# yellofi/SelectiveNet_for_semantic_segmentation_binary

Hardware: AMD Instinct MI355X
Metric: train images/sec, SelectiveUNet_B 256x256 bs=128 (global), selective_loss s_lamb=2 (higher is better)
Workload: dtype f32; 1 GPU; SelectiveUNet_B train step, global bs=128, 256x256, Adam lr=1e-3, s_lamb=2; model=SelectiveUNet_B, global_batch=128, per_gpu_batch=128, image=256, parallelism=dp1

## Files before the change

### selectivenet_for_semantic_segmentation_binary_amd/csrc/conv3x3.hip

```cpp
#include <cstdlib>

#include "gemm_common.h"

namespace selunet {

constexpr int TH = 16, TW = 16;
constexpr int HHT = TH + 2, HWT = TW + 2;
constexpr int HPIX = HHT * HWT;
constexpr int HTHREADS = 512;
constexpr int A_ROUNDS = (HPIX * 8 + HTHREADS - 1) / HTHREADS;
constexpr int AROWB = 160;
__device__ __forceinline__ int halo_off(int hp, int cc) { return hp * AROWB + ((cc ^ ((hp / HWT) & 1)) << 4); }

template <typename T, int BN, bool ONE_CHUNK>
__global__ void __launch_bounds__(HTHREADS, ONE_CHUNK ? 2 : 1)
conv3x3_halo_kernel(GatherArg g, const T* __restrict__ B, int N, int k_pad, EpiArg ep, int n_tiles, int tiles_x,
                    int tiles_y) {
  constexpr int E = 16 / sizeof(T);
  constexpr int CK = 128 / sizeof(T);
  constexpr int WAVES_N = BN / 64;
  constexpr int WAVES_M = 8 / WAVES_N;
  constexpr int WPIX = (TH * TW) / WAVES_M;
  constexpr int MT = WPIX / 32;
  constexpr int NT = 2;
// ... 290 lines not shown
        h[e] = a;
        l[e] = b;
      }
      const int par = (hp / HWT) & 1;
      *reinterpret_cast<f16x4*>(base + (((cc >> 1) ^ par) << 4) + (cc & 1) * 8) = h;
      *reinterpret_cast<f16x4*>(base + (((4 + (cc >> 1)) ^ par) << 4) + (cc & 1) * 8) = l;
    } else {
      *reinterpret_cast<uint4*>(base + (((cc ^ ((hp / HWT) & 1))) << 4)) = v;
    }
  };

  auto halo_store_prepped = [&](int hb, int hp, int cc, uint4 v) __attribute__((always_inline)) {
    unsigned char* base = As + hb * HPIX * AROWB + hp * AROWB;
    if constexpr (X2) {
      const int par = (hp / HWT) & 1;
      *reinterpret_cast<uint2*>(base + (((cc >> 1) ^ par) << 4) + (cc & 1) * 8) = make_uint2(v.x, v.y);
      *reinterpret_cast<uint2*>(base + (((4 + (cc >> 1)) ^ par) << 4) + (cc & 1) * 8) = make_uint2(v.z, v.w);
    } else {
      *reinterpret_cast<uint4*>(base + (((cc ^ ((hp / HWT) & 1))) << 4)) = v;
    }
  };
  auto tile_xy = [&](int pt_i, int& img, int& y0, int& x0) __attribute__((always_inline)) {
    const unsigned pt = (unsigned)pt_i;
    const unsigned r = pt / (unsigned)tiles_x;
    x0 = (int)(pt - r * (unsigned)tiles_x) * TW;
    const unsigned r2 = r / (unsigned)tiles_y;
    y0 = (int)(r - r2 * (unsigned)tiles_y) * TH;
    img = (int)r2;
  };
  auto a_slot = [&](int round, int& hp, int& cc) -> bool {
    const int hidx = round * HTHREADS + tid;
    hp = min(hidx >> 3, HPIX - 1);
    cc = hidx & 7;
    return hidx < HPIX * 8;
  };
  auto a_inside = [&](int y0, int x0, int hp) -> bool {
    const int hy = hp / HWT, hx = hp - (hp / HWT) * HWT;
    return (unsigned)(y0 - 1 + hy) < (unsigned)g.h && (unsigned)(x0 - 1 + hx) < (unsigned)g.w;
  };
  auto chunk_src = [&](int chunk, int& c) -> SrcArg {
    c = chunk * CK;
    const bool s1 = g.nsrc > 1 && c >= g.src[0].C;
    if (s1) c -= g.src[0].C;
    return pick_src(g, s1 ? 1 : 0);
  };
  auto a_ptr = [&](const SrcArg& sa, int c, int img, int y0, int x0, int hp, int cc) -> const uint4* {
    const int hy = hp / HWT, hx = hp - (hp / HWT) * HWT;
    const int ys = min(max(y0 - 1 + hy, 0), g.h - 1), xs = min(max(x0 - 1 + hx, 0), g.w - 1);
    return reinterpret_cast<const uint4*>(reinterpret_cast<const T*>(sa.data) +
                                          (((int64_t)img * g.h + ys) * g.w + xs) * sa.C + c + cc * E);
  };
  constexpr int XRPIX = 3 * HWT;
  static_assert(!X2 || (A_ROUNDS * 3 == HHT && XRPIX * 8 <= HTHREADS), "three halo rows per round");
  const int xq = tid >> 3, xcc = tid & 7;
  const int xhp = xq < XRPIX ? xq : xq - XRPIX;
  const int xry = (xhp >= HWT) + (xhp >= 2 * HWT), xhx = xhp - xry * HWT;
  const unsigned xpix = (unsigned)(xry * g.w + xhx);
  const unsigned xb_off = (unsigned)(xq * k_pad * 4 + xcc * 16);
  const unsigned xb_rstride = (unsigned)(64 * k_pad * 4);
  auto x_lds = [](int t) __attribute__((always_inline)) {
    const int q = t >> 3, cc = t & 7, hp = q < XRPIX ? q : q - XRPIX;
    const int ry = (hp >= HWT) + (hp >= 2 * HWT);
    return (unsigned)(hp * AROWB + (((cc >> 1) ^ (ry & 1)) << 4) + (cc & 1) * 8);
  };
  const unsigned xlds = x_lds(tid);
  unsigned xtb = 0;
  if constexpr (X2) {
    const int hrem = g.h - (tiles_y - 1) * TH, wrem = g.w - (tiles_x - 1) * TW;
#pragma unroll
    for (int r = 0; r < A_ROUNDS; ++r) {
      const int hy = 3 * r + xry;
      xtb |= (unsigned)((hy == 0) | (hy > hrem) << 6 | (xhx == 0) << 12 | (xhx > wrem) << 18) << r;
    }
  }
  struct Geo {
    int img, y0, x0;
    int64_t pix;
    unsigned em;
  };
  auto tile_geo = [&](int pt_) __attribute__((always_inline)) {
    const unsigned pt = (unsigned)__builtin_amdgcn_readfirstlane(pt_);
    const unsigned r = pt / (unsigned)tiles_x, tx = pt - r * (unsigned)tiles_x;
    const unsigned r2 = r / (unsigned)tiles_y, ty = r - r2 * (unsigned)tiles_y;
    Geo q;
    q.img = (int)r2;
    q.y0 = (int)ty * TH;
    q.x0 = (int)tx * TW;
    q.pix = ((int64_t)r2 * g.h + ty * TH) * g.w + tx * TW;
    q.em = (ty == 0 ? 0x3fu : 0u) | (ty == (unsigned)tiles_y - 1u ? 0x3fu << 6 : 0u) |
           (tx == 0 ? 0x3fu << 12 : 0u) | (tx == (unsigned)tiles_x - 1u ? 0x3fu << 18 : 0u);
    return q;
  };
  struct XStage {
    int64_t e0;
    unsigned off, rstride, safe, out;
  };
  auto x_stage = [&](const Geo& q, const SrcArg& sa, int c) __attribute__((always_inline)) {
    XStage s;
    s.e0 = (q.pix - g.w - 1) * sa.C + c;
    s.off = __umul24(xpix, (unsigned)sa.C * 4u) + (unsigned)xcc * 16u;
    s.rstride = (unsigned)(3 * g.w * sa.C) * 4u;
    s.safe = (unsigned)((g.w + 1) * sa.C) * 4u;
    s.out = xtb & q.em;
    return s;
  };
  auto x_out = [](const XStage& s, int r) __attribute__((always_inline)) { return (s.out & (0x41041u << r)) != 0; };
  auto at = [](const void* base, int64_t elems, unsigned off) __attribute__((always_inline)) {
    return reinterpret_cast<const uint4*>(
        reinterpret_cast<const char*>(reinterpret_cast<const float*>(base) + elems) + (size_t)off);
  };
  auto x_load = [&](const XStage& s, const SrcArg& sa, int r) __attribute__((always_inline)) {
    unsigned rs = (unsigned)r * s.rstride;
    asm volatile("" : "+s"(rs));
    return *at(sa.data, s.e0, x_out(s, r) ? s.safe : s.off + rs);
  };
  auto x_split4 = [&](uint4 v) __attribute__((always_inline)) {
#ifdef SELUNET_ABL_RAW_HALO
    return v;
#else
    float f[4];
    __builtin_memcpy(f, &v, 16);
    f16x4 h, l;
#pragma unroll
    for (int e = 0; e < 4; ++e) {
      _Float16 a, b;
      x2_split(f[e] * xs, a, b);
      h[e] = a;
      l[e] = b;
    }
    uint4 o;
    __builtin_memcpy(&o.x, &h, 8);
    __builtin_memcpy(&o.z, &l, 8);
    return o;
#endif
  };
  auto x_put = [&](int hb, int r, unsigned lds, uint4 o) __attribute__((always_inline)) {
    unsigned char* p = As + hb * HPIX * AROWB + r * (XRPIX * AROWB) + (lds ^ ((unsigned)(r & 1) << 4));
    *reinterpret_cast<uint2*>(p) = make_uint2(o.x, o.y);
    *reinterpret_cast<uint2*>(p + 64) = make_uint2(o.z, o.w);
  };
  struct BRegs {
    uint4 v[B_ROUNDS];
  };
  auto b_load = [&](int st) __attribute__((always_inline)) {
    const int chunk = st / 9, tap = st - chunk * 9;
    const int k0 = tap * g.Ctot + chunk * CK;
    BRegs rb;
    if constexpr (X2) {
      const int64_t e0 = (int64_t)n0 * k_pad + k0;
      unsigned o = xb_off;
      asm volatile("" : "+v"(o));
#pragma unroll
      for (int r = 0; r < B_ROUNDS; ++r) rb.v[r] = *at(B, e0, o + (unsigned)r * xb_rstride);
      return rb;
    }
#pragma unroll
    for (int r = 0; r < B_ROUNDS; ++r) {
      const int idx = r * HTHREADS + tid;
      const int row = idx >> 3, cc = idx & 7;
      rb.v[r] = *reinterpret_cast<const uint4*>(B + (int64_t)(n0 + row) * k_pad + k0 + cc * E);
    }
    return rb;
  };
  auto b_store = [&](const BRegs& rb, int buf) __attribute__((always_inline)) {
#pragma unroll
    for (int r = 0; r < B_ROUNDS; ++r) {
      const int idx = r * HTHREADS + tid;
      const int row = idx >> 3, cc = idx & 7;
      *reinterpret_cast<uint4*>(Bs + (buf * BN + row) * WROWB + cc * 16) = rb.v[r];
    }
  };

  AccT acc[AM][AN];
#pragma unroll
  for (int a = 0; a < AM; ++a)
#pragma unroll
    for (int b = 0; b < AN; ++b) acc[a][b] = AccT{};
  int hrow0[MT], hsw0[MT];
#pragma unroll
  for (int a = 0; a < MT; ++a) {
    const int pix = wm * WPIX + a * 32 + l32;
    hrow0[a] = (pix / TW) * HWT + (pix % TW);
    hsw0[a] = half ^ ((pix / TW) & 1);
  }
  auto mma_step = [&](int hbuf, int bbuf, int t) __attribute__((always_inline)) {
    const unsigned char* a_src = As + hbuf * HPIX * AROWB;
    const unsigned char* b_src = Bs + bbuf * BN * WROWB;
    const int dy = t / 3, dx = t - (t / 3) * 3;
    const int tap_off = dy * HWT + dx;
    if constexpr (M16) {
      f16x8 bh[4], bl[4];
#pragma unroll
      for (int b = 0; b < 4; ++b) {
        const unsigned char* p = b_src + (wn * 64 + b * 16 + l16) * WROWB + kg * 16;
        bh[b] = *reinterpret_cast<const f16x8*>(p);
        bl[b] = *reinterpret_cast<const f16x8*>(p + 64);
      }
#pragma unroll
      for (int a = 0; a < RT; ++a) {
        const int py = wm * RT + a;
        const unsigned char* p =
            a_src + ((py + dy) * HWT + l16 + dx) * AROWB + ((kg ^ ((py + dy) & 1)) << 4);
        const f16x8 ah = *reinterpret_cast<const f16x8*>(p);
        const f16x8 al = *reinterpret_cast<const f16x8*>(p + 64);
#pragma unroll
        for (int b = 0; b < 4; ++b) {
          acc[a][b] = __builtin_amdgcn_mfma_f32_16x16x32_f16(ah, bl[b], acc[a][b], 0, 0, 0);
          acc[a][b] = __builtin_amdgcn_mfma_f32_16x16x32_f16(al, bh[b], acc[a][b], 0, 0, 0);
          acc[a][b] = __builtin_amdgcn_mfma_f32_16x16x32_f16(ah, bh[b], acc[a][b], 0, 0, 0);
        }
      }
    } else if constexpr (X2) {
#pragma unroll
      for (int ks = 0; ks < 2; ++ks) {
        f16x8 ah[MT], al[MT], bh[NT], bl[NT];
#pragma unroll
        for (int a = 0; a < MT; ++a) {
          const unsigned char* p = a_src + (hrow0[a] + tap_off) * AROWB + ((hsw0[a] ^ dy) & 1) * 16;
          ah[a] = *reinterpret_cast<const f16x8*>(p + ks * 32);
          al[a] = *reinterpret_cast<const f16x8*>(p + (2 + ks) * 32);
        }
#pragma unroll
        for (int b = 0; b < NT; ++b) {
          const unsigned char* p = b_src + (wn * 64 + b * 32 + l32) * ROWB + half * 16;
          bh[b] = *reinterpret_cast<const f16x8*>(p + ks * 32);
          bl[b] = *reinterpret_cast<const f16x8*>(p + (2 + ks) * 32);
        }
#pragma unroll
        for (int a = 0; a < MT; ++a)
#pragma unroll
          for (int b = 0; b < NT; ++b) {
            acc[a][b] = __builtin_amdgcn_mfma_f32_32x32x16_f16(ah[a], bl[b], acc[a][b], 0, 0, 0);
            acc[a][b] = __builtin_amdgcn_mfma_f32_32x32x16_f16(al[a], bh[b], acc[a][b], 0, 0, 0);
            acc[a][b] = __builtin_amdgcn_mfma_f32_32x32x16_f16(ah[a], bh[b], acc[a][b], 0, 0, 0);
          }
      }
    } else {
#pragma unroll
      for (int q = 0; q < 4; ++q) {
        const int boff = q * 32 + half * 16;
        uint4 af[MT], bfr[NT];
#pragma unroll
        for (int a = 0; a < MT; ++a)
          af[a] = *reinterpret_cast<const uint4*>(a_src + (hrow0[a] + tap_off) * AROWB + q * 32 + ((hsw0[a] ^ dy) & 1) * 16);
#pragma unroll
        for (int b = 0; b < NT; ++b)
          bfr[b] = *reinterpret_cast<const uint4*>(b_src + (wn * 64 + b * 32 + l32) * WROWB + boff);
#pragma unroll
        for (int a = 0; a < MT; ++a)
#pragma unroll
          for (int b = 0; b < NT; ++b) Mma<T>::run(acc[a][b], af[a], bfr[b]);
      }
    }
  };
  auto halo_put_global = [&](uint4 v, int r, const SrcArg& sa, int c, int y0, int x0, int hb)
      __attribute__((always_inline)) {
    int hp, cc;
    if (!a_slot(r, hp, cc)) return;
    uint4 o = make_uint4(0, 0, 0, 0);
    if (a_inside(y0, x0, hp)) o = sa.scale ? transform16<T>(v, sa.scale, sa.shift, c + cc * E, sa.relu) : v;
    halo_store(hb, hp, cc, o);
  };

  Geo gc{}, gn{};
  if constexpr (X2) gc = gn = tile_geo(TQ ? pt_cur : prow);
  if (!TQ || pt_cur < ptiles) {
    int c0;
    const SrcArg sa = chunk_src(0, c0);
    uint4 v0[A_ROUNDS];
    if constexpr (X2) {
      const XStage s0 = x_stage(gc, sa, c0);
#pragma unroll
      for (int r = 0; r < A_ROUNDS; ++r) v0[r] = x_load(s0, sa, r);
#pragma unroll
      for (int r = 0; r < A_ROUNDS; ++r) {
        uint4 o = make_uint4(0, 0, 0, 0);
        if (!x_out(s0, r)) o = sa.scale ? transform16<T>(v0[r], sa.scale, sa.shift, c0 + xcc * E, sa.relu) : v0[r];
        x_put(0, r, xlds, x_split4(o));
      }
    } else {
      int img, y0, x0;
      tile_xy(TQ ? pt_cur : prow, img, y0, x0);
#pragma unroll
      for (int r = 0; r < A_ROUNDS; ++r) {
        int hp, cc;
        a_slot(r, hp, cc);
        v0[r] = *a_ptr(sa, c0, img, y0, x0, hp, cc);
      }
#pragma unroll
      for (int r = 0; r < A_ROUNDS; ++r) halo_put_global(v0[r], r, sa, c0, y0, x0, 0);
    }
  }
  BRegs rb_next = b_load(0);
  b_store(rb_next, 0);
  rb_next = b_load(1 % csteps);
  __syncthreads();

  using Acc = std::conditional_t<X2 && BN == 128, float, typename StatAcc<T>::type>;
  static_assert(stats_flush_bytes<BN, HTHREADS, Acc>() <= (int)sizeof(smem), "statistics scratch exceeds LDS");
  Acc s1[8] = {0, 0, 0, 0, 0, 0, 0, 0}, s2[8] = {0, 0, 0, 0, 0, 0, 0, 0}, s3[8] = {0, 0, 0, 0, 0, 0, 0, 0};
  float amx = 0.0f;
  const TileStats ts = tile_stats(ep, TQ ? 0 : prow, n0, N);
  float* tile = reinterpret_cast<float*>(smem);
  uint4 ra[A_ROUNDS];
  int J = 0;
  int S = 0;
  unsigned claimed = 0;
  for (int i = 0; TQ ? pt_cur < ptiles : i < ntl; ++i) {
    int img, y0, x0;
    if constexpr (X2) {
      img = gc.img, y0 = gc.y0, x0 = gc.x0;
      if constexpr (!TQ) gn = i + 1 < ntl ? tile_geo(prow + (i + 1) * gp) : gc;
    } else {
      tile_xy(TQ ? pt_cur : prow + i * gp, img, y0, x0);
    }
    BRegs rb_hold;
    for (int c = 0; c < nchunks; ++c, ++J) {
      if constexpr (TQ) {
        if (c == 1) {
          pt_next = tq_slot;
          gn = pt_next < ptiles ? tile_geo(pt_next) : gc;
        }
      }
      const bool last_c = c + 1 == nchunks;
      const bool has_next = !last_c || (TQ ? pt_next < ptiles : i + 1 < ntl);
      const bool defer = last_c && has_next;
      int nimg = img, ny0 = y0, nx0 = x0;
      if constexpr (!X2) {
        if (defer) tile_xy(TQ ? pt_next : prow + (i + 1) * gp, nimg, ny0, nx0);
      }
      const int nc = !has_next ? c : (last_c ? 0 : c + 1);
      int cs;
      const SrcArg sn = chunk_src(nc, cs);
      XStage sx{};
      if constexpr (X2) sx = x_stage(defer ? gn : gc, sn, cs);
      float* ssc = Ss + ((J + 1) & 1) * CK;
      float* ssh = Ss + 2 * CK + ((J + 1) & 1) * CK;
      float coef = 0.0f;
#pragma unroll
      for (int t = 0; t < 9; ++t) {
        const int st2 = c * 9 + t + 2;
        const BRegs rb_far = b_load(st2 < csteps ? st2 : st2 - csteps);
        if (t == 0 && sn.scale && tid < 2 * CK) coef = tid < CK ? sn.scale[cs + tid] : sn.shift[cs + tid - CK];
#pragma unroll
        for (int r = 0; r < A_ROUNDS; ++r) {
          if (halo_load_tap(r) == t) {
            if constexpr (X2) {
              ra[r] = x_load(sx, sn, r);
            } else {
              int hp, cc;
              a_slot(r, hp, cc);
              ra[r] = *a_ptr(sn, cs, nimg, ny0, nx0, hp, cc);
            }
          }
        }
        if constexpr (TQ) {
          if (c == 0 && t == 0 && tid == 0) claimed = atomicAdd(tq + n_tile, 1u);
        }
        mma_step(J & 1, S & 1, t);
        if constexpr (TQ) {
          if (c == 0 && t == 8 && tid == 0) tq_slot = (int)min(claimed, (unsigned)ptiles);
        }
        if (defer && t == 8) rb_hold = rb_next;
        else b_store(rb_next, (S + 1) & 1);
        if (t == 1 && sn.scale && tid < 2 * CK) (tid < CK ? ssc[tid] : ssh[tid - CK]) = coef;
#pragma unroll
        for (int r = 0; r < A_ROUNDS; ++r) {
          if (halo_write_tap(r) != t) continue;
          if constexpr (X2) {
            uint4 v = ra[r];
#ifndef SELUNET_ABL_RAW_HALO
            if (sn.scale) {
              float e[4];
              __builtin_memcpy(e, &v, 16);
#pragma unroll
              for (int j = 0; j < 4; ++j) {
                float f = e[j] * ssc[xcc * 4 + j] + ssh[xcc * 4 + j];
                if (sn.relu) f = fmaxf(f, 0.0f);
                e[j] = f;
              }
              __builtin_memcpy(&v, e, 16);
            }
            if (x_out(sx, r)) v = make_uint4(0, 0, 0, 0);
#endif
            const uint4 o = x_split4(v);
            if (!defer) x_put((J + 1) & 1, r, xlds, o);
            else ra[r] = o;
            continue;
          }
          int hp, cc;
          if (a_slot(r, hp, cc)) {
            uint4 v = make_uint4(0, 0, 0, 0);
            if (a_inside(ny0, nx0, hp)) {
              v = ra[r];
              if (sn.scale) {
                T e[E];
                __builtin_memcpy(e, &v, 16);
#pragma unroll
                for (int j = 0; j < E; ++j) {
                  float f = to_f(e[j]) * ssc[cc * E + j] + ssh[cc * E + j];
                  if (sn.relu) f = fmaxf(f, 0.0f);
                  e[j] = from_f<T>(f);
                }
                __builtin_memcpy(&v, e, 16);
              }
            }
            if (!defer) {
              halo_store((J + 1) & 1, hp, cc, v);
            } else {
              if constexpr (X2) {
                float f[4];
                __builtin_memcpy(f, &v, 16);
                f16x4 h, l;
#pragma unroll
                for (int e = 0; e < 4; ++e) {
                  _Float16 a, b;
                  x2_split(f[e] * xs, a, b);
                  h[e] = a;
                  l[e] = b;
                }
                __builtin_memcpy(&v.x, &h, 8);
                __builtin_memcpy(&v.z, &l, 8);
              }
              ra[r] = v;
            }
          }
        }
        __syncthreads();
        rb_next = rb_far;
        ++S;
      }
      if (defer) {
      }
    }

    if constexpr (X2) {
#pragma unroll
      for (int a = 0; a < AM; ++a)
#pragma unroll
        for (int b = 0; b < AN; ++b) acc[a][b] *= cfac[b];
    }
    if constexpr (M16) {
#pragma unroll
      for (int a = 0; a < RT; ++a)
#pragma unroll
        for (int b = 0; b < 4; ++b)
#pragma unroll
          for (int i = 0; i < 4; ++i)
            tile[(wm * WPIX + a * 16 + 4 * kg + i) * (BN + 4) + wn * 64 + b * 16 + l16] = acc[a][b][i];
    } else {
      acc_to_lds<MT, NT, BN>(tile, acc, wm * WPIX, wn * 64, lane);
    }
#pragma unroll
    for (int a = 0; a < AM; ++a)
#pragma unroll
      for (int b = 0; b < AN; ++b) acc[a][b] = AccT{};
    __syncthreads();
    auto dst = [&](int pix, int cl) -> T* {
      const int y = y0 + pix / TW, x = x0 + pix % TW;
      if (y >= g.h || x >= g.w) return nullptr;
      const int64_t m = ((int64_t)img * g.h + y) * g.w + x;
      const int col = n0 + cl;
      if (ep.mode == SELUNET_EP_SPLIT)
        return col < ep.split ? reinterpret_cast<T*>(ep.out0) + m * ep.split + col
                              : reinterpret_cast<T*>(ep.out1) + m * (N - ep.split) + (col - ep.split);
      return reinterpret_cast<T*>(ep.out0) + m * N + col;
    };
    auto bias_col = [&](int cl) { return n0 + cl; };
    if constexpr (TQ) {
      TileStats tt = tile_stats(ep, pt_cur, n0, N);
      lds_tile_store_acc<T, TH * TW, BN, HTHREADS>(tile, tid, dst, ep.bias, bias_col, tt, s1, s2, s3, amx);
      tt.amax = nullptr;
      tile_stats_flush<BN, HTHREADS>(tile, tid, tt, s1, s2, s3, 0.0f);
#pragma unroll
      for (int e = 0; e < 8; ++e) s1[e] = s2[e] = s3[e] = 0;
    } else {
      lds_tile_store_acc<T, TH * TW, BN, HTHREADS>(tile, tid, dst, ep.bias, bias_col, ts, s1, s2, s3, amx);
    }
    if (TQ ? pt_next < ptiles : i + 1 < ntl) {
      __syncthreads();
      int tid2 = tid;
      asm volatile("" : "+v"(tid2));
#pragma unroll
      for (int r = 0; r < A_ROUNDS; ++r) {
        if constexpr (X2) {
          x_put(J & 1, r, x_lds(tid2), ra[r]);
        } else {
          const int hidx = r * HTHREADS + tid2;
          if (hidx < HPIX * 8) halo_store_prepped(J & 1, hidx >> 3, hidx & 7, ra[r]);
        }
      }
      b_store(rb_hold, S & 1);
      __syncthreads();
    }
    if constexpr (TQ) pt_cur = pt_next;
    gc = gn;
  }
  if constexpr (TQ) {
    if (ts.amax) block_amax(ts.amax, amx, tile);
    if (tid == 0 && atomicAdd(tq + n_tiles + n_tile, 1u) == (unsigned)gp - 1u) {
      atomicExch(tq + n_tile, 0u);
      atomicExch(tq + n_tiles + n_tile, 0u);
    }
  } else {
    tile_stats_flush<BN, HTHREADS>(tile, tid, ts, s1, s2, s3, amx);
  }
}

constexpr int WINO_STEPS = 12;
__device__ __forceinline__ int wino_row(int hp) {
  const int hy = hp / HWT, hx = hp - hy * HWT;
  return hy * HWT + (hx & 1) * (HWT / 2) + (hx >> 1);
}

template <int BN, int XS>
__global__ void __launch_bounds__(HTHREADS, 1)
conv3x3_wino_persist_kernel(GatherArg g, const float* __restrict__ B, int N, int k_pad, EpiArg ep, int n_tiles,
                            int tiles_x, int tiles_y, int ptiles, int gp) {
  using T = float;
  constexpr int E = 4;
  constexpr int CK = 32;
  constexpr int NT = BN / 64;
  constexpr int STEPS = WINO_STEPS / XS;
  constexpr int BROWS = XS * BN;
  constexpr int B_ROUNDS = BROWS * 8 / HTHREADS;
  static_assert(XS == 1 || XS == 2, "one or two planes per step");
  auto lt = [](int r) { return XS == 1 ? r : r >> 1; };
  static_assert(B_ROUNDS * HTHREADS == BROWS * 8, "weight tile rows must split evenly over the threads");
  static_assert(A_ROUNDS <= 6, "halo slice schedule covers six slices");

  constexpr int SMEM_MAIN = 2 * HPIX * AROWB + 2 * BROWS * ROWB + 2 * CK * 8;
  constexpr int SMEM_EPI = TH * TW * (BN + 4) * 4;
  __shared__ __attribute__((aligned(16))) unsigned char smem[SMEM_MAIN > SMEM_EPI ? SMEM_MAIN : SMEM_EPI];
  unsigned char* As = smem;
  unsigned char* Bs = smem + 2 * HPIX * AROWB;
  float* Ss = reinterpret_cast<float*>(Bs + 2 * BROWS * ROWB);

  const int tid = threadIdx.x;
  const int lane = tid & 63, wave = tid >> 6;
  const int wm = wave >> 1, wn = wave & 1;
  const int half = lane >> 5, l32 = lane & 31;
  const int pair = wm * 32 + l32, py = pair >> 3, px2 = pair & 7;

  const unsigned lb = xcd_remap(blockIdx.x, gridDim.x);
  const int n_tile = lb % n_tiles;
  const int prow = lb / n_tiles;
  const int n0 = n_tile * BN;
  const int ntl = prow < ptiles ? (ptiles - prow + gp - 1) / gp : 0;
  const int nchunks = g.Ctot / CK;
  const int csteps = nchunks * STEPS;

  auto tile_xy = [&](int i, int& img, int& y0, int& x0) __attribute__((always_inline)) {
    const unsigned pt = (unsigned)(prow + i * gp);
    const unsigned r = pt / (unsigned)tiles_x;
    x0 = (int)(pt - r * (unsigned)tiles_x) * TW;
    const unsigned r2 = r / (unsigned)tiles_y;
    y0 = (int)(r - r2 * (unsigned)tiles_y) * TH;
    img = (int)r2;
  };
  auto a_slot = [&](int round, int& hp, int& cc) -> bool {
    const int hidx = round * HTHREADS + tid;
    hp = min(hidx >> 3, HPIX - 1);
    cc = hidx & 7;
    return hidx < HPIX * 8;
  };
  auto a_inside = [&](int y0, int x0, int hp) -> bool {
    const int hy = hp / HWT, hx = hp - (hp / HWT) * HWT;
    return (unsigned)(y0 - 1 + hy) < (unsigned)g.h && (unsigned)(x0 - 1 + hx) < (unsigned)g.w;
  };
  auto chunk_src = [&](int chunk, int& c) -> SrcArg {
    c = chunk * CK;
    const bool s1 = g.nsrc > 1 && c >= g.src[0].C;
    if (s1) c -= g.src[0].C;
    return pick_src(g, s1 ? 1 : 0);
  };
  auto a_ptr = [&](const SrcArg& sa, int c, int img, int y0, int x0, int hp, int cc) -> const uint4* {
    const int hy = hp / HWT, hx = hp - (hp / HWT) * HWT;
    const int ys = min(max(y0 - 1 + hy, 0), g.h - 1), xs = min(max(x0 - 1 + hx, 0), g.w - 1);
    return reinterpret_cast<const uint4*>(reinterpret_cast<const T*>(sa.data) +
                                          (((int64_t)img * g.h + ys) * g.w + xs) * sa.C + c + cc * E);
  };
  struct BRegs {
    uint4 v[B_ROUNDS];
  };
  auto b_load = [&](int st) __attribute__((always_inline)) {
    const int chunk = st / STEPS, t = st - chunk * STEPS;
    BRegs rb;
#pragma unroll
    for (int r = 0; r < B_ROUNDS; ++r) {
      const int idx = r * HTHREADS + tid;
      const int row = idx >> 3, cc = idx & 7;
      const int pl = row / BN, co = row - pl * BN;
      const int k0 = (t * XS + pl) * g.Ctot + chunk * CK;
      rb.v[r] = *reinterpret_cast<const uint4*>(B + (int64_t)(n0 + co) * k_pad + k0 + cc * E);
    }
    return rb;
  };
  auto b_store = [&](const BRegs& rb, int buf) __attribute__((always_inline)) {
#pragma unroll
    for (int r = 0; r < B_ROUNDS; ++r) {
      const int idx = r * HTHREADS + tid;
      const int row = idx >> 3, cc = idx & 7;
      *reinterpret_cast<uint4*>(Bs + (buf * BROWS + row) * ROWB + cc * 16) = rb.v[r];
    }
  };

  f32x16 acc[4][NT];
#pragma unroll
  for (int x = 0; x < 4; ++x)
#pragma unroll
    for (int b = 0; b < NT; ++b) acc[x][b] = f32x16{};
  const int prow0 = py * HWT + px2;

  auto mma_step = [&](int hbuf, int bbuf, int t) __attribute__((always_inline)) {
    const unsigned char* a_src = As + hbuf * HPIX * AROWB;
    const unsigned char* b_src = Bs + bbuf * BROWS * ROWB;
    const int dy = (t * XS) >> 2, x0i = (t * XS) & 3;
    const int sw = ((half ^ (py + dy)) & 1) * 16;
    auto drow = [&](int j) { return a_src + (prow0 + dy * HWT + (j & 1) * (HWT / 2) + (j >> 1)) * AROWB + sw; };
#pragma unroll
    for (int q = 0; q < 4; ++q) {
      uint4 bfr[XS][NT];
#pragma unroll
      for (int p = 0; p < XS; ++p)
#pragma unroll
        for (int b = 0; b < NT; ++b)
          bfr[p][b] = *reinterpret_cast<const uint4*>(b_src + (p * BN + wn * (BN / 2) + b * 32 + l32) * ROWB + q * 32 +
                                                      half * 16);
      float4 v[XS];
      if (XS == 1) {
        const int xi = x0i;
        const int ja = xi == 0 ? 0 : (xi == 2 ? 2 : 1);
        const int jb = xi == 3 ? 3 : (xi == 2 ? 1 : 2);
        const float4 da = *reinterpret_cast<const float4*>(drow(ja) + q * 32);
        const float4 db = *reinterpret_cast<const float4*>(drow(jb) + q * 32);
        v[0] = xi == 1 ? make_float4(da.x + db.x, da.y + db.y, da.z + db.z, da.w + db.w)
                       : make_float4(da.x - db.x, da.y - db.y, da.z - db.z, da.w - db.w);
      } else {
        const int j0 = x0i == 0 ? 0 : 1;
        const float4 e0 = *reinterpret_cast<const float4*>(drow(j0) + q * 32);
        const float4 e1 = *reinterpret_cast<const float4*>(drow(j0 + 1) + q * 32);
        const float4 e2 = *reinterpret_cast<const float4*>(drow(j0 + 2) + q * 32);
        if (x0i == 0) {
          v[0] = make_float4(e0.x - e2.x, e0.y - e2.y, e0.z - e2.z, e0.w - e2.w);
          v[XS - 1] = make_float4(e1.x + e2.x, e1.y + e2.y, e1.z + e2.z, e1.w + e2.w);
        } else {
          v[0] = make_float4(e1.x - e0.x, e1.y - e0.y, e1.z - e0.z, e1.w - e0.w);
          v[XS - 1] = make_float4(e0.x - e2.x, e0.y - e2.y, e0.z - e2.z, e0.w - e2.w);
        }
      }
#pragma unroll
      for (int p = 0; p < XS; ++p) {
        const uint4 av = make_uint4(__float_as_uint(v[p].x), __float_as_uint(v[p].y), __float_as_uint(v[p].z),
                                    __float_as_uint(v[p].w));
#pragma unroll
        for (int b = 0; b < NT; ++b) Mma<float>::run(acc[x0i + p][b], av, bfr[p][b]);
      }
    }
  };
  auto halo_put_global = [&](uint4 v, int r, const SrcArg& sa, int c, int y0, int x0, int hb)
      __attribute__((always_inline)) {
    int hp, cc;
    if (!a_slot(r, hp, cc)) return;
    uint4 o = make_uint4(0, 0, 0, 0);
    if (a_inside(y0, x0, hp)) o = sa.scale ? transform16<T>(v, sa.scale, sa.shift, c + cc * E, sa.relu) : v;
    *reinterpret_cast<uint4*>(As + hb * HPIX * AROWB + halo_off(wino_row(hp), cc)) = o;
  };

  {
    int img, y0, x0;
    tile_xy(0, img, y0, x0);
    int c0;
    const SrcArg sa = chunk_src(0, c0);
    uint4 v0[A_ROUNDS];
#pragma unroll
    for (int r = 0; r < A_ROUNDS; ++r) {
      int hp, cc;
      a_slot(r, hp, cc);
      v0[r] = *a_ptr(sa, c0, img, y0, x0, hp, cc);
    }
#pragma unroll
    for (int r = 0; r < A_ROUNDS; ++r) halo_put_global(v0[r], r, sa, c0, y0, x0, 0);
  }
  BRegs rb_next = b_load(0);
  b_store(rb_next, 0);
  rb_next = b_load(1 % csteps);
  __syncthreads();

  using Acc = std::conditional_t<BN == 128, float, typename StatAcc<T>::type>;
  static_assert(stats_flush_bytes<BN, HTHREADS, Acc>() <= (int)sizeof(smem), "statistics scratch exceeds LDS");
  Acc s1[8] = {0, 0, 0, 0, 0, 0, 0, 0}, s2[8] = {0, 0, 0, 0, 0, 0, 0, 0}, s3[8] = {0, 0, 0, 0, 0, 0, 0, 0};
  float amx = 0.0f;
  const TileStats ts = tile_stats(ep, prow, n0, N);
  float* tile = reinterpret_cast<float*>(smem);
  uint4 ra[A_ROUNDS];
  int J = 0;
  int S = 0;
  for (int i = 0; i < ntl; ++i) {
    int img, y0, x0;
    tile_xy(i, img, y0, x0);
    BRegs rb_hold;
    for (int c = 0; c < nchunks; ++c, ++J) {
      const bool last_c = c + 1 == nchunks;
      const bool has_next = !last_c || i + 1 < ntl;
      const bool defer = last_c && has_next;
      int nimg = img, ny0 = y0, nx0 = x0;
      if (defer) tile_xy(i + 1, nimg, ny0, nx0);
      const int nc = !has_next ? c : (last_c ? 0 : c + 1);
      int cs;
      const SrcArg sn = chunk_src(nc, cs);
      float* ssc = Ss + ((J + 1) & 1) * CK;
      float* ssh = Ss + 2 * CK + ((J + 1) & 1) * CK;
      float coef = 0.0f;
#pragma unroll
      for (int t = 0; t < STEPS; ++t) {
        const int st2 = c * STEPS + t + 2;
        const BRegs rb_far = b_load(st2 < csteps ? st2 : st2 - csteps);
        if (t == 0 && !defer && sn.scale && tid < 2 * CK) coef = tid < CK ? sn.scale[cs + tid] : sn.shift[cs + tid - CK];
#pragma unroll
        for (int r = 0; r < A_ROUNDS; ++r) {
          if (lt(r) == t) {
            int hp, cc;
            a_slot(r, hp, cc);
            ra[r] = *a_ptr(sn, cs, nimg, ny0, nx0, hp, cc);
          }
        }
        mma_step(J & 1, S & 1, t);
        if (defer && t == STEPS - 1) rb_hold = rb_next;
        else b_store(rb_next, (S + 1) & 1);
        if (!defer) {
          if (t == 1 && sn.scale && tid < 2 * CK) (tid < CK ? ssc[tid] : ssh[tid - CK]) = coef;
#pragma unroll
          for (int r = 0; r < A_ROUNDS; ++r) {
            if (lt(r) + 3 != t) continue;
            int hp, cc;
            if (a_slot(r, hp, cc)) {
              uint4 v = make_uint4(0, 0, 0, 0);
              if (a_inside(ny0, nx0, hp)) {
                v = ra[r];
                if (sn.scale) {
                  float e[E];
                  __builtin_memcpy(e, &v, 16);
#pragma unroll
                  for (int j = 0; j < E; ++j) {
                    float f = e[j] * ssc[cc * E + j] + ssh[cc * E + j];
                    if (sn.relu) f = fmaxf(f, 0.0f);
                    e[j] = f;
                  }
                  __builtin_memcpy(&v, e, 16);
                }
              }
              *reinterpret_cast<uint4*>(As + ((J + 1) & 1) * HPIX * AROWB + halo_off(wino_row(hp), cc)) = v;
            }
          }
        }
        __syncthreads();
        rb_next = rb_far;
        ++S;
      }
    }

#pragma unroll
    for (int b = 0; b < NT; ++b) {
      const int col = wn * (BN / 2) + b * 32 + l32;
#pragma unroll
      for (int r = 0; r < 16; ++r) {
        const int pr = wm * 32 + (r & 3) + 8 * (r >> 2) + 4 * half;
        const int e = (pr >> 3) * TW + 2 * (pr & 7);
        const float m0 = acc[0][b][r], m1 = acc[1][b][r], m2 = acc[2][b][r], m3 = acc[3][b][r];
        tile[e * (BN + 4) + col] = (m0 + m1) + m2;
        tile[(e + 1) * (BN + 4) + col] = (m1 - m2) - m3;
      }
    }
#pragma unroll
    for (int x = 0; x < 4; ++x)
#pragma unroll
      for (int b = 0; b < NT; ++b) acc[x][b] = f32x16{};
    __syncthreads();
    auto dst = [&](int pix, int cl) -> T* {
      const int y = y0 + pix / TW, x = x0 + pix % TW;
// ... 1420 lines not shown
```

### selectivenet_for_semantic_segmentation_binary_amd/csrc/gemm_common.h

```cpp
#pragma once

#include <type_traits>

#include "common.h"

namespace selunet {

struct SrcArg {
  const void* data;
  const float* scale;
  const float* shift;
  int C;
  int relu;
  int layout;
  int pad;
};

struct GatherArg {
  int n, h, w;
  int taps;
  int nsrc;
  int Ctot;
  int hs, ws;
  int K;
  int small;
  int64_t M;
  SrcArg src[2];
};

__device__ __forceinline__ SrcArg pick_src(const GatherArg& g, int s) {
  SrcArg r;
  r.data = s ? g.src[1].data : g.src[0].data;
  r.scale = s ? g.src[1].scale : g.src[0].scale;
  r.shift = s ? g.src[1].shift : g.src[0].shift;
  r.C = s ? g.src[1].C : g.src[0].C;
  r.relu = s ? g.src[1].relu : g.src[0].relu;
  r.layout = s ? g.src[1].layout : g.src[0].layout;
  r.pad = 0;
  return r;
}

constexpr int BM = SELUNET_GEMM_BM;
constexpr int ROWB = 144;

__device__ __forceinline__ void tap_offset(int taps, int tap, int& dy, int& dx) {
  if (taps == 9) {
    dy = tap / 3 - 1;
    dx = tap - (tap / 3) * 3 - 1;
  } else if (taps == 4) {
    dy = tap >> 1;
    dx = tap & 1;
  } else {
    dy = 0;
    dx = 0;
  }
}

__device__ __forceinline__ bool src_pixel(const GatherArg& g, int tap, int y, int x, int& ys, int& xs) {
  int dy, dx;
  tap_offset(g.taps, tap, dy, dx);
  if (g.taps == 4) {
    ys = 2 * y + dy;
    xs = 2 * x + dx;
    return true;
  }
  ys = y + dy;
  xs = x + dx;
  return (unsigned)ys < (unsigned)g.hs && (unsigned)xs < (unsigned)g.ws;
}

__device__ __forceinline__ int64_t src_index(const GatherArg& g, int64_t m, int tap) {
  if (g.taps == 1) return m;
  const unsigned mu = (unsigned)m;
  const unsigned x = mu % (unsigned)g.w, t = mu / (unsigned)g.w;
  const unsigned y = t % (unsigned)g.h, img = t / (unsigned)g.h;
  int ys, xs;
  if (!src_pixel(g, tap, (int)y, (int)x, ys, xs)) return -1;
  return ((int64_t)img * g.hs + ys) * g.ws + xs;
}

template <typename T>
__device__ __forceinline__ float gather_scalar(const GatherArg& g, int64_t m, int k) {
  if (m >= g.M || k >= g.K) return 0.0f;
  const int tap = k / g.Ctot;
  int c = k - tap * g.Ctot;
  int s = 0;
  if (g.nsrc > 1 && c >= g.src[0].C) {
    c -= g.src[0].C;
    s = 1;
  }
  const int x = (int)(m % g.w);
  const int64_t t = m / g.w;
  const int y = (int)(t % g.h);
  const int img = (int)(t / g.h);
  int ys, xs;
  if (!src_pixel(g, tap, y, x, ys, xs)) return 0.0f;
  const SrcArg sa = pick_src(g, s);
  float v;
  if (sa.layout == 1) {
    v = reinterpret_cast<const float*>(sa.data)[(((int64_t)img * sa.C + c) * g.hs + ys) * g.ws + xs];
  } else {
    v = to_f(reinterpret_cast<const T*>(sa.data)[(((int64_t)img * g.hs + ys) * g.ws + xs) * sa.C + c]);
  }
  if (sa.scale) {
    v = v * sa.scale[c] + sa.shift[c];
    if (sa.relu) v = fmaxf(v, 0.0f);
  }
  return v;
}

template <typename T> struct Mma;
template <> struct Mma<float> {
  __device__ static inline void run(f32x16& acc, uint4 a, uint4 b) {
    acc = __builtin_amdgcn_mfma_f32_32x32x2f32(__uint_as_float(a.x), __uint_as_float(b.x), acc, 0, 0, 0);
    acc = __builtin_amdgcn_mfma_f32_32x32x2f32(__uint_as_float(a.y), __uint_as_float(b.y), acc, 0, 0, 0);
    acc = __builtin_amdgcn_mfma_f32_32x32x2f32(__uint_as_float(a.z), __uint_as_float(b.z), acc, 0, 0, 0);
    acc = __builtin_amdgcn_mfma_f32_32x32x2f32(__uint_as_float(a.w), __uint_as_float(b.w), acc, 0, 0, 0);
  }
};
template <> struct Mma<__bf16> {
  __device__ static inline void run(f32x16& acc, uint4 a, uint4 b) {
    bf16x8 av = __builtin_bit_cast(bf16x8, a);
    bf16x8 bv = __builtin_bit_cast(bf16x8, b);
    acc = __builtin_amdgcn_mfma_f32_32x32x16_bf16(av, bv, acc, 0, 0, 0);
  }
};

template <typename T>
__device__ __forceinline__ uint4 transform16(uint4 raw, const float* scale, const float* shift, int c, int relu) {
  constexpr int E = 16 / sizeof(T);
  T v[E];
  __builtin_memcpy(v, &raw, 16);
#pragma unroll
  for (int e = 0; e < E; ++e) {
    float f = to_f(v[e]) * scale[c + e] + shift[c + e];
    if (relu) f = fmaxf(f, 0.0f);
    v[e] = from_f<T>(f);
  }
  uint4 out;
  __builtin_memcpy(&out, v, 16);
  return out;
}

struct BnBwdArg {
  const void* y;
  const float* scale;
  const float* shift;
  const float* mean;
  const float* invstd;
  float* slab;
};

struct EpiArg {
  void* out0;
  void* out1;
  const float* bias;
  float* stats;
  int mode;
  int split;
  float* colsum;
  BnBwdArg bnb;
  float* amax;
  const float* stats_center;
};

typedef short s16x4 __attribute__((ext_vector_type(4)));

__device__ __forceinline__ unsigned xcd_remap(unsigned b, unsigned nb) {
  const unsigned xcd = b & 7u, q = nb >> 3, r = nb & 7u;
  const unsigned base = xcd < r ? xcd * (q + 1) : r * (q + 1) + (xcd - r) * q;
  return base + (b >> 3);
}

template <int MT, int NT, int TC>
__device__ __forceinline__ void acc_to_lds(float* tile, const f32x16 (&acc)[MT][NT], int wr0, int wc0, int lane) {
  const int half = lane >> 5, l32 = lane & 31;
#pragma unroll
  for (int a = 0; a < MT; ++a)
#pragma unroll
    for (int b = 0; b < NT; ++b)
#pragma unroll
      for (int r = 0; r < 16; ++r)
        tile[(wr0 + a * 32 + (r & 3) + 8 * (r >> 2) + 4 * half) * (TC + 4) + wc0 + b * 32 + l32] = acc[a][b][r];
}

struct TileStats {
  float* stats;
  int ld;
  float* colsum;
  int colsum_cols;
  int gcol0;
  BnBwdArg bnb;
  const void* out0;
  float* amax;
  const float* center;
};

__device__ __forceinline__ TileStats tile_stats(const EpiArg& ep, int64_t row, int n0, int N) {
  TileStats ts;
  ts.ld = N;
  ts.stats = ep.stats ? ep.stats + row * 2 * N + n0 : nullptr;
  ts.colsum = ep.colsum ? ep.colsum + row * ep.split + n0 : nullptr;
  ts.colsum_cols = ep.split;
  ts.gcol0 = n0;
  ts.bnb = ep.bnb;
  if (ep.bnb.slab) {
    ts.bnb.scale += n0;
    ts.bnb.shift += n0;
    ts.bnb.mean += n0;
    ts.bnb.invstd += n0;
    ts.bnb.slab += row * 3 * N + n0;
  }
  ts.out0 = ep.out0;
  ts.amax = ep.amax;
  ts.center = ep.stats_center ? ep.stats_center + n0 : nullptr;
  return ts;
}

template <typename T> struct StatAcc { using type = float; };
template <> struct StatAcc<float> { using type = double; };

template <typename T, int TR, int TC, int NTHREADS, typename Dst, typename BiasCol, typename Acc>
__device__ __forceinline__ void lds_tile_store_acc(float* tile, int tid, Dst&& dst, const float* bias,
                                                   BiasCol&& bias_col, const TileStats& ts, Acc (&s1)[8],
                                                   Acc (&s2)[8], Acc (&s3)[8], float& am) {
  constexpr int CC = TC / 8;
  constexpr int RS = NTHREADS / CC;
  asm volatile("" : "+v"(tid));
  const int cc = tid % CC, r0 = tid / CC;
  const int col = cc * 8;
  float bv[8], cen[8];
#pragma unroll
  for (int e = 0; e < 8; ++e) bv[e] = bias ? bias[bias_col(col + e)] : 0.0f;
  const bool do_st = ts.stats != nullptr;
#pragma unroll
  for (int e = 0; e < 8; ++e) cen[e] = do_st && ts.center ? ts.center[col + e] : 0.0f;
  const bool do_cs = ts.colsum != nullptr && ts.gcol0 + col < ts.colsum_cols;
  const bool do_bn = ts.bnb.slab != nullptr;
  float sc[8], sh[8], mu[8], is[8];
  if (do_bn) {
#pragma unroll
    for (int e = 0; e < 8; ++e) {
      sc[e] = ts.bnb.scale[col + e];
      sh[e] = ts.bnb.shift[col + e];
      mu[e] = ts.bnb.mean[col + e];
      is[e] = ts.bnb.invstd[col + e];
    }
  }
  __builtin_amdgcn_s_waitcnt(0x0F70);
  constexpr bool WIDE = !std::is_same<Acc, float>::value;
  float tw1[WIDE ? 8 : 1] = {}, tw2[WIDE ? 8 : 1] = {}, tw3[WIDE ? 8 : 1] = {};
  float* t1 = WIDE ? tw1 : reinterpret_cast<float*>(s1);
  float* t2 = WIDE ? tw2 : reinterpret_cast<float*>(s2);
  float* t3 = WIDE ? tw3 : reinterpret_cast<float*>(s3);
  constexpr int NR = TR / RS;
  constexpr int YB = NR < (TC >= 128 ? 4 : 2) ? NR : (TC >= 128 ? 4 : 2);
  static_assert(TR % RS == 0 && NR % YB == 0, "epilogue rows must split evenly over the threads");
#pragma unroll 1
  for (int rb = 0; rb < NR; rb += YB) {
  T yb[YB][8];
  if (do_bn) {
#pragma unroll
    for (int j = 0; j < YB; ++j) {
      const T* p = dst(r0 + (rb + j) * RS, col);
      if (p == nullptr) continue;
      const T* yp = reinterpret_cast<const T*>(ts.bnb.y) + (p - reinterpret_cast<const T*>(ts.out0));
      if constexpr (sizeof(T) == 2) {
        const uint4 u = *reinterpret_cast<const uint4*>(yp);
        __builtin_memcpy(yb[j], &u, 16);
      } else {
        const f32x4 a = *reinterpret_cast<const f32x4*>(yp), b = *reinterpret_cast<const f32x4*>(yp + 4);
        __builtin_memcpy(yb[j], &a, 16);
        __builtin_memcpy(yb[j] + 4, &b, 16);
      }
    }
  }
#pragma unroll
  for (int j = 0; j < YB; ++j) {
    const int row = r0 + (rb + j) * RS;
    T* p = dst(row, col);
    if (p == nullptr) continue;
    const f32x4 lo = *reinterpret_cast<const f32x4*>(tile + row * (TC + 4) + col);
    const f32x4 hi = *reinterpret_cast<const f32x4*>(tile + row * (TC + 4) + col + 4);
    float v[8] = {lo[0], lo[1], lo[2], lo[3], hi[0], hi[1], hi[2], hi[3]};
    if (do_st) {
#pragma unroll
      for (int e = 0; e < 8; ++e) {
        const float d = v[e] - cen[e];
        t1[e] += d;
        t2[e] += d * d;
      }
    }
#pragma unroll
    for (int e = 0; e < 8; ++e) v[e] += bv[e];
    T o[8];
#pragma unroll
    for (int e = 0; e < 8; ++e) o[e] = from_f<T>(v[e]);
    if (ts.amax) {
#pragma unroll
      for (int e = 0; e < 8; ++e) am = fmaxf(am, fabsf(to_f(o[e])));
    }
    if constexpr (sizeof(T) == 2) {
      uint4 u;
      __builtin_memcpy(&u, o, 16);
      *reinterpret_cast<uint4*>(p) = u;
    } else {
      *reinterpret_cast<f32x4*>(p) = f32x4{v[0], v[1], v[2], v[3]};
      *reinterpret_cast<f32x4*>(p + 4) = f32x4{v[4], v[5], v[6], v[7]};
    }
    if (do_cs) {
#pragma unroll
      for (int e = 0; e < 8; ++e) t1[e] += to_f(o[e]);
    }
    if (do_bn) {
#pragma unroll
      for (int e = 0; e < 8; ++e) {
        const float y = to_f(yb[j][e]);
        const float da = y * sc[e] + sh[e] > 0.0f ? to_f(o[e]) : 0.0f;
        const float xh = (y - mu[e]) * is[e];
        t1[e] += da;
        t2[e] += da * xh;
        t3[e] += xh;
      }
    }
  }
  }
  if constexpr (WIDE) {
#pragma unroll
    for (int e = 0; e < 8; ++e) {
      s1[e] += (Acc)t1[e];
      s2[e] += (Acc)t2[e];
      s3[e] += (Acc)t3[e];
    }
  }
}

template <int TC, int NTHREADS, typename Acc>
constexpr int stats_flush_bytes() { return (NTHREADS / (TC / 8)) * TC * 3 * (int)sizeof(Acc); }

template <int TC, int NTHREADS, typename Acc>
__device__ __forceinline__ void tile_stats_flush(float* red_f, int tid, const TileStats& ts, const Acc (&s1)[8],
                                                 const Acc (&s2)[8], const Acc (&s3)[8], float am) {
  constexpr int CC = TC / 8;
  constexpr int RS = NTHREADS / CC;
  Acc* red = reinterpret_cast<Acc*>(red_f);
  const int cc = tid % CC, r0 = tid / CC;
  const int col = cc * 8;
  const bool do_st = ts.stats != nullptr;
  const bool do_bn = ts.bnb.slab != nullptr;
  const int nst = do_bn ? 3 : (do_st ? 2 : 1);
  if (do_st || ts.colsum != nullptr || do_bn) {
    __syncthreads();
#pragma unroll
    for (int e = 0; e < 8; ++e) {
      red[(r0 * TC + col + e) * 3 + 0] = s1[e];
      red[(r0 * TC + col + e) * 3 + 1] = s2[e];
      red[(r0 * TC + col + e) * 3 + 2] = s3[e];
    }
    __syncthreads();
    for (int i = tid; i < TC * nst; i += NTHREADS) {
      const int c = i % TC, k = i / TC;
      Acc a = 0;
      for (int r = 0; r < RS; ++r) a += red[(r * TC + c) * 3 + k];
      if (do_bn) ts.bnb.slab[k * ts.ld + c] = a;
      else if (do_st) ts.stats[k * ts.ld + c] = a;
      else if (ts.gcol0 + c < ts.colsum_cols) ts.colsum[c] = a;
    }
  }
  if (ts.amax) block_amax(ts.amax, am, red_f);
}

template <typename T, int TR, int TC, int NTHREADS, typename Dst, typename BiasCol>
__device__ __forceinline__ void lds_tile_store(float* tile, int tid, Dst&& dst, const float* bias, BiasCol&& bias_col,
                                               const TileStats& ts) {
  float s1[8] = {0, 0, 0, 0, 0, 0, 0, 0}, s2[8] = {0, 0, 0, 0, 0, 0, 0, 0}, s3[8] = {0, 0, 0, 0, 0, 0, 0, 0};
  float am = 0.0f;
  lds_tile_store_acc<T, TR, TC, NTHREADS>(tile, tid, dst, bias, bias_col, ts, s1, s2, s3, am);
  tile_stats_flush<TC, NTHREADS>(tile, tid, ts, s1, s2, s3, am);
}

int make_gather(const selunet_gather* a, int dtype, GatherArg& g, int vec_elems);

bool conv3x3_halo_eligible(const GatherArg& g, int N, int dtype);
int64_t conv3x3_halo_tiles(const GatherArg& g);
int64_t conv3x3_halo_stats_rows(const GatherArg& g, int N, int dtype);
bool conv3x3_halo_one_chunk(const GatherArg& g, int dtype);
bool conv3x3_halo_persistent(const GatherArg& g, int dtype);
int conv3x3_halo_launch(const GatherArg& g, const void* b, int N, int k_pad, const EpiArg& ep, int dtype,
                        hipStream_t st);
bool conv3x3_wino_shape_ok(int h, int w, int c_in, int c_src0, int n_cols);
bool conv3x3_wgrad_wino_eligible(const GatherArg& p, const GatherArg& q, int dtype);
int64_t conv3x3_wgrad_wino_splits(const GatherArg& p, const GatherArg& q);
int conv3x3_wgrad_wino_launch(const GatherArg& p, const GatherArg& q, float* ws, int ldw, hipStream_t st);
bool conv3x3_wino_eligible(const GatherArg& g, int N);
bool conv3x3_bn128(int N, const EpiArg& ep, int split_mult);
int conv3x3_wino_launch(const GatherArg& g, const float* u, int N, const EpiArg& ep, hipStream_t st);
bool conv3x3_x2_shape_ok(int h, int w, int c_in, int c_src0, int n_cols);
bool conv3x3_x2_eligible(const GatherArg& g, int N);
int conv3x3_x2_launch(const GatherArg& g, const float* w, int N, const EpiArg& ep, const float* amax0,
                      const float* amax1, hipStream_t st);
bool convt_x2_eligible(const GatherArg& g, int N, const EpiArg& e);
int convt_dgrad_x2_ntb(const GatherArg& g, int N);
int64_t convt_dgrad_x2_rows(const GatherArg& g, int N);
bool convt_dgrad_x2_eligible(const GatherArg& g, int N, const EpiArg& e);
int convt_dgrad_x2_launch(const GatherArg& g, const float* w, int N, const EpiArg& e, const float* amax_src,
                          hipStream_t st);
bool convt_ring_dgrad_operand_ok(const GatherArg& g, int N);
int64_t convt_ring_rows(const GatherArg& g, int N);
bool convt_ring_x2_takes(const GatherArg& g, int N, const EpiArg& e);
int convt_ring_x2_launch(const GatherArg& g, const float* w, int N, const EpiArg& e, const float* amax_src,
                         hipStream_t st);
bool convt_ring_bf16_dgrad_operand_ok(const GatherArg& g, int N);
bool convt_ring_bf16_takes(const GatherArg& g, int N, const EpiArg& e);
int convt_ring_bf16_launch(const GatherArg& g, const void* w, int N, const EpiArg& e, hipStream_t st);
int convt_bf16_fwd_ntb(const GatherArg& g, int N);
int convt_dgrad_bf16_ntb(const GatherArg& g, int N);
int64_t convt_dgrad_bf16_rows(const GatherArg& g, int N);
bool convt_bf16_eligible(const GatherArg& g, int N, const EpiArg& e);
bool convt_dgrad_bf16_eligible(const GatherArg& g, int N, const EpiArg& e);
int convt_bf16_launch(const GatherArg& g, const void* w, int N, const EpiArg& e, hipStream_t st);
int convt_x2_launch(const GatherArg& g, const float* w, int N, const EpiArg& e, const float* amax_src,
                    hipStream_t st);
int64_t conv3x3_persist_rows(const GatherArg& g, int N);
int conv3x3_persist_wgs();
bool conv3x3_x2d_eligible(const GatherArg& g, int N);
int64_t conv3x3_x2d_rows(const GatherArg& g);
int conv3x3_x2d_launch(const GatherArg& g, const float* w, const EpiArg& ep, const float* amax0, const float* amax1,
                       hipStream_t st);
bool conv3x3_wgrad_halo_eligible(const GatherArg& p, const GatherArg& q, int dtype);
int64_t conv3x3_wgrad_x2_splits(const GatherArg& p, const GatherArg& q);
bool x2_tile_queue();
bool conv3x3_x2p_eligible(const GatherArg& g, int N);
int64_t conv3x3_x2p_rows(const GatherArg& g, int N);
int conv3x3_x2p_launch(const GatherArg& g, const float* w, int N, const EpiArg& ep, const float* amax0,
                       const float* amax1, hipStream_t st);
int64_t conv3x3_x2_persist_rows(const GatherArg& g, int N);
struct WgradBnArg {
  const float* y;
  const float* scale;
  const float* shift;
  const float* mean;
  const float* invstd;
  const float* coef;
  float* dy;
  float* dy_amax;
  int kind;
  int nh;
  const float* pooled;
  const float* skip;
  const float* hw;
  const float* g0;
  const float* g1;
  const float* g2;
};
int conv3x3_wgrad_x2_launch(const GatherArg& p, const GatherArg& q, float* ws, int ldo, const float* amax_p,
                            const float* amax_q0, const float* amax_q1, hipStream_t st,
                            const WgradBnArg* bn = nullptr);
int conv3x3_wgrad_halo_launch(const GatherArg& p, const GatherArg& q, float* out, int ldo, float* ws, int dtype,
                              hipStream_t st);
int64_t conv3x3_wgrad_halo_splits(const GatherArg& p, const GatherArg& q, int dtype);
bool halo_enabled();

}
```

Measured before the change: 1436 images/s.

## Stage epilogue coefficients in LDS and batch y loads in X2 conv epilogue

```diff
diff --git a/selectivenet_for_semantic_segmentation_binary_amd/csrc/conv3x3.hip b/selectivenet_for_semantic_segmentation_binary_amd/csrc/conv3x3.hip
--- a/selectivenet_for_semantic_segmentation_binary_amd/csrc/conv3x3.hip
+++ b/selectivenet_for_semantic_segmentation_binary_amd/csrc/conv3x3.hip
@@ -616,6 +616,13 @@
   float amx = 0.0f;
   const TileStats ts = tile_stats(ep, TQ ? 0 : prow, n0, N);
   float* tile = reinterpret_cast<float*>(smem);
+  constexpr int EPI_YB = X2 ? 4 : 0;
+  float* ecoef = nullptr;
+  if constexpr (X2) {
+    __shared__ __attribute__((aligned(16))) float ecoef_s[EPI_COEF_ROWS * BN];
+    ecoef = ecoef_s;
+    epi_coef_stage<BN, HTHREADS>(ecoef, tid, ep.bias, [&](int cl) { return n0 + cl; }, ts);
+  }
   uint4 ra[A_ROUNDS];
   int J = 0;
   int S = 0;
@@ -783,13 +790,13 @@
     auto bias_col = [&](int cl) { return n0 + cl; };
     if constexpr (TQ) {
       TileStats tt = tile_stats(ep, pt_cur, n0, N);
-      lds_tile_store_acc<T, TH * TW, BN, HTHREADS>(tile, tid, dst, ep.bias, bias_col, tt, s1, s2, s3, amx);
+      lds_tile_store_acc<T, TH * TW, BN, HTHREADS, EPI_YB>(tile, tid, dst, ep.bias, bias_col, tt, s1, s2, s3, amx, ecoef);
       tt.amax = nullptr;
       tile_stats_flush<BN, HTHREADS>(tile, tid, tt, s1, s2, s3, 0.0f);
 #pragma unroll
       for (int e = 0; e < 8; ++e) s1[e] = s2[e] = s3[e] = 0;
     } else {
-      lds_tile_store_acc<T, TH * TW, BN, HTHREADS>(tile, tid, dst, ep.bias, bias_col, ts, s1, s2, s3, amx);
+      lds_tile_store_acc<T, TH * TW, BN, HTHREADS, EPI_YB>(tile, tid, dst, ep.bias, bias_col, ts, s1, s2, s3, amx, ecoef);
     }
     if (TQ ? pt_next < ptiles : i + 1 < ntl) {
       __syncthreads();
diff --git a/selectivenet_for_semantic_segmentation_binary_amd/csrc/gemm_common.h b/selectivenet_for_semantic_segmentation_binary_amd/csrc/gemm_common.h
--- a/selectivenet_for_semantic_segmentation_binary_amd/csrc/gemm_common.h
+++ b/selectivenet_for_semantic_segmentation_binary_amd/csrc/gemm_common.h
@@ -220,12 +220,150 @@
 template <typename T> struct StatAcc { using type = float; };
 template <> struct StatAcc<float> { using type = double; };
 
-template <typename T, int TR, int TC, int NTHREADS, typename Dst, typename BiasCol, typename Acc>
+constexpr int EPI_COEF_ROWS = 6;
+
+template <int TC, int NTHREADS, typename BiasCol>
+__device__ __forceinline__ void epi_coef_stage(float* coef, int tid, const float* bias, BiasCol&& bias_col,
+                                               const TileStats& ts) {
+  for (int i = tid; i < EPI_COEF_ROWS * TC; i += NTHREADS) {
+    const int k = i / TC, c = i - k * TC;
+    float v = 0.0f;
+    if (k == 0) {
+      if (bias) v = bias[bias_col(c)];
+    } else if (k == 1) {
+      if (ts.stats != nullptr && ts.center) v = ts.center[c];
+    } else if (ts.bnb.slab != nullptr) {
+      v = (k == 2 ? ts.bnb.scale : k == 3 ? ts.bnb.shift : k == 4 ? ts.bnb.mean : ts.bnb.invstd)[c];
+    }
+    coef[i] = v;
+  }
+}
+
+template <typename T, int TR, int TC, int NTHREADS, int CYB = 0, typename Dst, typename BiasCol, typename Acc>
 __device__ __forceinline__ void lds_tile_store_acc(float* tile, int tid, Dst&& dst, const float* bias,
                                                    BiasCol&& bias_col, const TileStats& ts, Acc (&s1)[8],
-                                                   Acc (&s2)[8], Acc (&s3)[8], float& am) {
+                                                   Acc (&s2)[8], Acc (&s3)[8], float& am,
+                                                   const float* coef = nullptr) {
   constexpr int CC = TC / 8;
   constexpr int RS = NTHREADS / CC;
+  if constexpr (CYB > 0) {
+    constexpr int NR = TR / RS, NB = NR / CYB;
+    static_assert(TR % RS == 0 && NR % CYB == 0, "epilogue rows must split evenly over the threads");
+    asm volatile("" : "+v"(tid));
+    const int cc = tid % CC, r0 = tid / CC;
+    const int col = cc * 8;
+    const bool do_st = ts.stats != nullptr;
+    const bool do_cs = ts.colsum != nullptr && ts.gcol0 + col < ts.colsum_cols;
+    const bool do_bn = ts.bnb.slab != nullptr;
+    T yb[CYB][8];
+    auto y_load = [&](int b) __attribute__((always_inline)) {
+#pragma unroll
+      for (int j = 0; j < CYB; ++j) {
+        const T* p = dst(r0 + (b * CYB + j) * RS, col);
+        if (p == nullptr) p = dst(0, col);
+        const T* yp = reinterpret_cast<const T*>(ts.bnb.y) + (p - reinterpret_cast<const T*>(ts.out0));
+        T* yr = yb[j];
+        if constexpr (sizeof(T) == 2) {
+          const uint4 u = *reinterpret_cast<const uint4*>(yp);
+          __builtin_memcpy(yr, &u, 16);
+        } else {
+          const f32x4 a = *reinterpret_cast<const f32x4*>(yp), c = *reinterpret_cast<const f32x4*>(yp + 4);
+          __builtin_memcpy(yr, &a, 16);
+          __builtin_memcpy(yr + 4, &c, 16);
+        }
+      }
+    };
+    auto coef8 = [&](int k, float (&o)[8]) __attribute__((always_inline)) {
+      const f32x4 a = *reinterpret_cast<const f32x4*>(coef + k * TC + col);
+      const f32x4 c = *reinterpret_cast<const f32x4*>(coef + k * TC + col + 4);
+      __builtin_memcpy(o, &a, 16);
+      __builtin_memcpy(o + 4, &c, 16);
+    };
+    constexpr bool WIDE = !std::is_same<Acc, float>::value;
+    float tw1[WIDE ? 8 : 1] = {}, tw2[WIDE ? 8 : 1] = {}, tw3[WIDE ? 8 : 1] = {};
+    float* t1 = WIDE ? tw1 : reinterpret_cast<float*>(s1);
+    float* t2 = WIDE ? tw2 : reinterpret_cast<float*>(s2);
+    float* t3 = WIDE ? tw3 : reinterpret_cast<float*>(s3);
+    float bv[8], cen[8], sc[8], sh[8], mu[8], is[8];
+    auto row_pass = [&](auto bnb, int row, const T* yr) __attribute__((always_inline)) {
+      constexpr bool BNB = decltype(bnb)::value;
+      T* p = dst(row, col);
+      if (p == nullptr) return;
+      const f32x4 lo = *reinterpret_cast<const f32x4*>(tile + row * (TC + 4) + col);
+      const f32x4 hi = *reinterpret_cast<const f32x4*>(tile + row * (TC + 4) + col + 4);
+      float v[8] = {lo[0], lo[1], lo[2], lo[3], hi[0], hi[1], hi[2], hi[3]};
+      if constexpr (!BNB) {
+        if (do_st) {
+#pragma unroll
+          for (int e = 0; e < 8; ++e) {
+            const float d = v[e] - cen[e];
+            t1[e] += d;
+            t2[e] += d * d;
+          }
+        }
+      }
+#pragma unroll
+      for (int e = 0; e < 8; ++e) v[e] += BNB ? 0.0f : bv[e];
+      T o[8];
+#pragma unroll
+      for (int e = 0; e < 8; ++e) o[e] = from_f<T>(v[e]);
+      if (ts.amax) {
+#pragma unroll
+        for (int e = 0; e < 8; ++e) am = fmaxf(am, fabsf(to_f(o[e])));
+      }
+      if constexpr (sizeof(T) == 2) {
+        uint4 u;
+        __builtin_memcpy(&u, o, 16);
+        *reinterpret_cast<uint4*>(p) = u;
+      } else {
+        *reinterpret_cast<f32x4*>(p) = f32x4{v[0], v[1], v[2], v[3]};
+        *reinterpret_cast<f32x4*>(p + 4) = f32x4{v[4], v[5], v[6], v[7]};
+      }
+      if constexpr (!BNB) {
+        if (do_cs) {
+#pragma unroll
+          for (int e = 0; e < 8; ++e) t1[e] += to_f(o[e]);
+        }
+      } else {
+#pragma unroll
+        for (int e = 0; e < 8; ++e) {
+          const float y = to_f(yr[e]);
+          const float da = y * sc[e] + sh[e] > 0.0f ? to_f(o[e]) : 0.0f;
+          const float xh = (y - mu[e]) * is[e];
+          t1[e] += da;
+          t2[e] += da * xh;
+          t3[e] += xh;
+        }
+      }
+    };
+    if (do_bn) {
+      coef8(2, sc);
+      coef8(3, sh);
+      coef8(4, mu);
+      coef8(5, is);
+      __builtin_amdgcn_s_waitcnt(0x0F70);
+#pragma unroll 1
+      for (int b = 0; b < NB; ++b) {
+        y_load(b);
+#pragma unroll
+        for (int j = 0; j < CYB; ++j) row_pass(std::true_type{}, r0 + (b * CYB + j) * RS, yb[j]);
+      }
+    } else {
+      coef8(0, bv);
+      coef8(1, cen);
+#pragma unroll
+      for (int j = 0; j < NR; ++j) row_pass(std::false_type{}, r0 + j * RS, nullptr);
+    }
+    if constexpr (WIDE) {
+#pragma unroll
+      for (int e = 0; e < 8; ++e) {
+        s1[e] += (Acc)t1[e];
+        s2[e] += (Acc)t2[e];
+        s3[e] += (Acc)t3[e];
+      }
+    }
+    return;
+  }
   asm volatile("" : "+v"(tid));
   const int cc = tid % CC, r0 = tid / CC;
   const int col = cc * 8;
```

After: 1442 images/s (median of 6 runs). No clear change (+0.4%).
